# octavian-ganea/equidock_public

Measured on NVIDIA H100. Metric: protein_pairs_per_sec_iegmn_fwd_kabsch, higher is better.
Workload: dtype f32

## Files before the change

### equidock_public_b200/csrc/edge_stage_tc.cu

```cuda
#include "tc_common.cuh"

namespace eqd {
#define TC_WGS 3
#define TC_THREADS (128 * TC_WGS)
#define TC_ROWS 64
#define TC_MAX_TN 32
#define TC_LD 72
#define TC_W_BYTES 67584
#define TC_W1_SPLIT 6144
#define TC_W23_BASE 18432
#define TC_W23_SPLIT 16384
#define TC_HE_FLOATS (TC_ROWS * EQD_EDGE_FEATS + 16)
#define TC_A_SPLIT 6144

struct __align__(128) TcWgSmem {
  unsigned char a[3 * TC_A_SPLIT];
  float msg[TC_ROWS * TC_LD];
  float he[TC_HE_FLOATS];
  double xs[2][TC_ROWS * 6];
  double xm[TC_ROWS * 3];
  double phi[TC_ROWS];
  int src[2][TC_ROWS];
  int dst[2][TC_ROWS];
  int rp[2][TC_MAX_TN + 4];
  unsigned long long he_bar;
};

struct EdgeConsts {
  float ln_g[64], ln_b[64], b2[64], b3[64], w4[64];
};

struct TcSmem {
  unsigned char w[TC_W_BYTES];
  TcWgSmem wg[TC_WGS];
  EdgeConsts cst;
  unsigned long long w_bar;
};

__global__ void __launch_bounds__(TC_THREADS, 1)
edge_stage_tc_kernel(eqd_graph g, eqd_layer_params p, const __grid_constant__ EdgeConsts cst_p,
                     const float* __restrict__ proj, const double* __restrict__ x_in, const double* __restrict__ x_orig,
                     float* __restrict__ aggr, double* __restrict__ x_out, int* __restrict__ status, int tn) {
  extern __shared__ __align__(128) unsigned char smem_raw[];
  TcSmem& S = *reinterpret_cast<TcSmem*>(smem_raw);
  const int tid = threadIdx.x, wgi = tid >> 7, t = tid & 127, r = t & 63, half = t >> 6;
  const int warp = t >> 5, lane = t & 31;
  TcWgSmem& W = S.wg[wgi];
  const EdgeConsts& cst = S.cst;
  const int bar = 1 + wgi;
  const int pw = 128 + 3 * p.dhp;
  const int ntiles = (g.n_nodes + tn - 1) / tn;
  const float slope = p.leaky_slope;

  TRACE_START(0);
  if (tid == 0) {
    mbar_init(&S.w_bar, 1);
    for (int w = 0; w < TC_WGS; ++w) mbar_init(&S.wg[w].he_bar, 1);
    asm volatile("fence.mbarrier_init.release.cluster;" ::: "memory");
    mbar_expect_tx(&S.w_bar, TC_W_BYTES);
    bulk_g2s(S.w, p.w_edge_tc, TC_W_BYTES, &S.w_bar);
  }
  for (int i = tid; i < 5 * 64; i += TC_THREADS) (&S.cst.ln_g[0])[i] = (&cst_p.ln_g[0])[i];
  __syncthreads();
  mbar_wait(&S.w_bar, 0);
  unsigned he_phase = 0;
  const unsigned w_saddr = smem_u32(S.w), a_saddr = smem_u32(W.a);
  auto a_desc = [&](int sp, int kb) { return a_desc_at<TC_ROWS>(a_saddr, TC_A_SPLIT, 0, sp, kb); };

  auto prefetch = [&](int tile, int buf, int e0, int e1, int& off_l, int& n_l, int& off_r) {
    const int n0 = tile * tn, nn = min(tn, g.n_nodes - n0);
    const int ne = e1 - e0;
    off_l = off_r = 0;
    n_l = 0;
    if (ne <= TC_ROWS) {
      if (r < ne) {
        if (half == 0) cp_async4(&W.src[buf][r], g.col_src + e0 + r);
        else cp_async4(&W.dst[buf][r], g.edge_dst + e0 + r);
      }
      if (half == 0 && r <= nn) cp_async4(&W.rp[buf][r], g.row_ptr + n0 + r);
      const int el0 = min(e0, g.n_lig_edges), el1 = min(e1, g.n_lig_edges);
      n_l = el1 - el0;
      long sl = 0, sr = 0;
      unsigned bl = 0, br = 0;
      if (n_l > 0) {
        long b0 = (long)el0 * (EQD_EDGE_FEATS * 4), b1 = (long)el1 * (EQD_EDGE_FEATS * 4);
        sl = b0 & ~15L;
        bl = (unsigned)(((b1 + 15) & ~15L) - sl);
        off_l = (int)((b0 - sl) >> 2);
      }
      const int nr = ne - n_l;
      const unsigned dst_r_off = bl;
      if (nr > 0) {
        long b0 = (long)(e0 + n_l - g.n_lig_edges) * (EQD_EDGE_FEATS * 4), b1 = (long)(e1 - g.n_lig_edges) * (EQD_EDGE_FEATS * 4);
        sr = b0 & ~15L;
        br = (unsigned)(((b1 + 15) & ~15L) - sr);
        off_r = (int)(dst_r_off >> 2) + (int)((b0 - sr) >> 2);
      }
      if (t == 0) {
        mbar_expect_tx(&W.he_bar, bl + br);
        if (bl) bulk_g2s(W.he, reinterpret_cast<const unsigned char*>(g.he_lig) + sl, bl, &W.he_bar);
        if (br) bulk_g2s(reinterpret_cast<unsigned char*>(W.he) + dst_r_off, reinterpret_cast<const unsigned char*>(g.he_rec) + sr, br,
                         &W.he_bar);
      }
    }
    cp_async_commit();
  };
  auto prefetch_x = [&](int b, int ne_t) {
    if (r < ne_t && ne_t <= TC_ROWS) {
      const double* xp = x_in + (long)(half == 0 ? W.src[b][r] : W.dst[b][r]) * 3;
#pragma unroll
      for (int c = 0; c < 3; ++c) cp_async8(&W.xs[b][r * 6 + half * 3 + c], xp + c);
    }
    cp_async_commit();
  };
  auto row_range = [&](int tile, int& e0, int& e1) {
    const int n0 = tile * tn;
    e0 = __ldg(g.row_ptr + n0);
    e1 = __ldg(g.row_ptr + n0 + min(tn, g.n_nodes - n0));
  };

  int tile = blockIdx.x * TC_WGS + wgi;
  const int tstride = gridDim.x * TC_WGS;
  int buf = 0;
  int e0 = 0, ne = 0, off_l = 0, n_l = 0, off_r = 0;
  if (tile < ntiles) {
    int e1;
    row_range(tile, e0, e1);
    ne = e1 - e0;
    prefetch(tile, buf, e0, e1, off_l, n_l, off_r);
    cp_async_wait<0>();
    prefetch_x(buf, ne);
  }
  const int fr0 = warp * 16 + (lane >> 2), fc = 2 * (lane & 3);

  for (; tile < ntiles; tile += tstride) {
    const int n0 = tile * tn, nn = min(tn, g.n_nodes - n0);
    const bool has_next = tile + tstride < ntiles;
    int e0n = 0, e1n = 0, off_ln = 0, n_ln = 0, off_rn = 0;
    if (has_next) row_range(tile + tstride, e0n, e1n);
    const int nen = e1n - e0n;
    if (ne > TC_ROWS) {
      if (t == 0) atomicOr(status + g.n_pairs, EQD_STATUS_DEGREE_OVERFLOW);
      cp_async_wait<0>();
      wg_barrier(bar);
      if (has_next) {
        prefetch(tile + tstride, buf ^ 1, e0n, e1n, off_ln, n_ln, off_rn);
        cp_async_wait<0>();
        prefetch_x(buf ^ 1, nen);
      }
      e0 = e0n; ne = nen; off_l = off_ln; n_l = n_ln; off_r = off_rn; buf ^= 1;
      continue;
    }
    if (t == 0) TRACE_PHASE(0, blockIdx.x * TC_WGS + wgi, tile, 2);
    const int o_upd = 127 - t;
    const int nd_upd = o_upd / 3, comp_upd = o_upd - nd_upd * 3;
    const long gi_upd = (long)(n0 + nd_upd) * 3 + comp_upd;
    double xo_upd = 0.0, xi_upd = 0.0;
    if (o_upd < nn * 3) {
      xo_upd = x_orig[gi_upd];
      xi_upd = x_in[gi_upd];
    }
    cp_async_wait<0>();
    wg_barrier(bar);
    float2 ps[16], pd[16];
#pragma unroll
    for (int h = 0; h < 2; ++h) {
      const int fr = fr0 + 8 * h;
      const bool ok = fr < ne;
      const float* sp = proj + (long)(ok ? W.src[buf][fr] : 0) * pw + fc;
      const float* dp = proj + (long)(ok ? W.dst[buf][fr] : n0) * pw + 64 + fc;
#pragma unroll
      for (int j = 0; j < 8; ++j) {
        ps[2 * j + h] = __ldg(reinterpret_cast<const float2*>(sp + 8 * j));
        pd[2 * j + h] = __ldg(reinterpret_cast<const float2*>(dp + 8 * j));
      }
    }
    const bool valid = r < ne;
    {
      float a1v[24];
      mbar_wait(&W.he_bar, he_phase);
      he_phase ^= 1;
      const float* hrow = W.he + (r < n_l ? off_l + r * EQD_EDGE_FEATS : off_r + (r - n_l) * EQD_EDGE_FEATS);
      if (half == 0) {
#pragma unroll
        for (int k = 0; k < 24; ++k) a1v[k] = valid ? hrow[k] : 0.f;
      } else {
        double rx = 0.0, ry = 0.0, rz = 0.0;
        if (valid) {
          const double* xs = W.xs[buf] + r * 6;
          rx = xs[0] - xs[3];
          ry = xs[1] - xs[4];
          rz = xs[2] - xs[5];
          W.xm[r * 3 + 0] = rx;
          W.xm[r * 3 + 1] = ry;
          W.xm[r * 3 + 2] = rz;
        }
#pragma unroll
        for (int k = 0; k < 3; ++k) a1v[k] = valid ? hrow[24 + k] : 0.f;
        const float nd2 = valid ? -(float)(rx * rx + ry * ry + rz * rz) : -INFINITY;
        constexpr double kS[EQD_N_RBF] = {1.0, 1.5, 2.25, 3.375, 5.0625, 7.59375, 11.390625, 17.0859375, 25.62890625,
                                          38.443359375, 57.6650390625, 86.49755859375, 129.746337890625,
                                          194.6195068359375, 291.92926025390625};
#pragma unroll
        for (int j = 0; j < EQD_N_RBF; ++j)
          a1v[3 + j] = exp2f(nd2 * (float)(1.4426950408889634 / kS[j]));
#pragma unroll
        for (int k = 18; k < 24; ++k) a1v[k] = 0.f;
      }
      unsigned p0[12], p1[12], p2[12];
#pragma unroll
      for (int c = 0; c < 12; ++c) split3_pair(a1v[2 * c], a1v[2 * c + 1], p0[c], p1[c], p2[c]);
#pragma unroll
      for (int j = 0; j < 3; ++j) a_store8<TC_ROWS>(W.a, TC_A_SPLIT, r, half * 24 + 8 * j, p0 + 4 * j, p1 + 4 * j, p2 + 4 * j);
    }
    tc_fence_before();
    const bool deg10 = wg_barrier_and(bar, t >= nn || W.rp[buf][t + 1] - W.rp[buf][t] == 10);
    unsigned af[3][4][4];
    {
      float v[32];
      wg_gemm6_issue<64>(v, a_desc, [&](int sp, int kb) { return b_desc_ex(w_saddr + sp * TC_W1_SPLIT + kb * 2048, 1024, 128); },
                         3, false);
      if (has_next) prefetch(tile + tstride, buf ^ 1, e0n, e1n, off_ln, n_ln, off_rn);
      wg_mma_wait(v);
#pragma unroll
      for (int h = 0; h < 2; ++h)
#pragma unroll
        for (int j = 0; j < 8; ++j) {
          float& x0 = v[4 * j + 2 * h];
          float& x1 = v[4 * j + 2 * h + 1];
          x0 = __fadd_rn(__fadd_rn(x0, ps[2 * j + h].x), pd[2 * j + h].x);
          x1 = __fadd_rn(__fadd_rn(x1, ps[2 * j + h].y), pd[2 * j + h].y);
          x0 = fmaxf(x0, __fmul_rn(x0, slope));
          x1 = fmaxf(x1, __fmul_rn(x1, slope));
        }
      float pv[32];
#pragma unroll
      for (int i = 0; i < 32; ++i) pv[i] = __shfl_xor_sync(0xffffffffu, v[i], 2);
      float mean[2], rstd[2];
#pragma unroll
      for (int h = 0; h < 2; ++h) {
        float mh[2], qh[2];
#pragma unroll
        for (int ch = 0; ch < 2; ++ch) {
          float s0 = 0.f, s1 = 0.f;
#pragma unroll
          for (int c4 = 0; c4 < 8; ++c4) {
            s0 = __fadd_rn(s0, chain_val(v, pv, h, ch, c4, 0));
            s1 = __fadd_rn(s1, chain_val(v, pv, h, ch, c4, 1));
          }
          const float sp = s0 + s1;
          mh[ch] = (sp + __shfl_xor_sync(0xffffffffu, sp, 1)) * (1.f / 32.f);
          float q0 = 0.f, q1 = 0.f;
#pragma unroll
          for (int c4 = 0; c4 < 8; ++c4) {
            const float d0 = __fadd_rn(chain_val(v, pv, h, ch, c4, 0), -mh[ch]);
            const float d1 = __fadd_rn(chain_val(v, pv, h, ch, c4, 1), -mh[ch]);
            q0 = fmaf(d0, d0, q0);
            q1 = fmaf(d1, d1, q1);
          }
          const float qp = q0 + q1;
          qh[ch] = qp + __shfl_xor_sync(0xffffffffu, qp, 1);
        }
        const float m0 = mh[0], m1 = mh[1];
        mean[h] = 0.5f * (m0 + m1);
        const float dm = m0 - m1;
        const float var = (qh[0] + qh[1] + dm * dm * 16.f) * (1.f / 64.f);
        rstd[h] = 1.f / sqrtf(var + 1e-5f);
      }
#pragma unroll
      for (int j = 0; j < 8; ++j) {
        const float2 gj = *reinterpret_cast<const float2*>(&cst.ln_g[8 * j + fc]);
        const float2 bj = *reinterpret_cast<const float2*>(&cst.ln_b[8 * j + fc]);
#pragma unroll
        for (int h = 0; h < 2; ++h) {
          float& x0 = v[4 * j + 2 * h];
          float& x1 = v[4 * j + 2 * h + 1];
          x0 = fmaf(__fmul_rn(__fadd_rn(x0, -mean[h]), rstd[h]), gj.x, bj.x);
          x1 = fmaf(__fmul_rn(__fadd_rn(x1, -mean[h]), rstd[h]), gj.y, bj.y);
        }
      }
      acc_to_a_split3<4>(v, af);
    }
    if (has_next) {
      cp_async_wait<0>();
      prefetch_x(buf ^ 1, nen);
    }
    {
      auto w23 = [&](int hn) {
        return [&, hn](int sp, int kb) {
          return b_desc_ex(w_saddr + TC_W23_BASE + sp * TC_W23_SPLIT + kb * 4096 + hn * 1024, 2048, 128); };
      };
      float m[32], hd[32];
      wg_gemm6_rs_issue<64>(m, af, w23(0), false);
      wg_gemm6_rs_issue<64>(hd, af, w23(1), false);
      wg_mma_wait(m);
      wg_mma_wait(hd);
      float u[32];
#pragma unroll
      for (int j = 0; j < 8; ++j) {
        const float2 b2 = *reinterpret_cast<const float2*>(&cst.b2[8 * j + fc]);
        const float2 b3 = *reinterpret_cast<const float2*>(&cst.b3[8 * j + fc]);
#pragma unroll
        for (int h = 0; h < 2; ++h) {
          *reinterpret_cast<float2*>(W.msg + (fr0 + 8 * h) * TC_LD + 8 * j + fc) =
              make_float2(__fadd_rn(m[4 * j + 2 * h], b2.x), __fadd_rn(m[4 * j + 2 * h + 1], b2.y));
          const float x0 = __fadd_rn(hd[4 * j + 2 * h], b3.x), x1 = __fadd_rn(hd[4 * j + 2 * h + 1], b3.y);
          u[4 * j + 2 * h] = fmaxf(x0, __fmul_rn(x0, slope));
          u[4 * j + 2 * h + 1] = fmaxf(x1, __fmul_rn(x1, slope));
        }
      }
      float pu[32];
#pragma unroll
      for (int i = 0; i < 32; ++i) pu[i] = __shfl_xor_sync(0xffffffffu, u[i], 2);
      double phv[2];
#pragma unroll
      for (int h = 0; h < 2; ++h) {
        double red[2];
#pragma unroll
        for (int ch = 0; ch < 2; ++ch) {
          const float* w4 = cst.w4 + 32 * ch + 2 * (lane & 1);
          float p0 = 0.f, p1 = 0.f;
#pragma unroll
          for (int c4 = 0; c4 < 8; ++c4) {
            p0 = fmaf(chain_val(u, pu, h, ch, c4, 0), w4[4 * c4], p0);
            p1 = fmaf(chain_val(u, pu, h, ch, c4, 1), w4[4 * c4 + 1], p1);
          }
          const double pp = (double)p0 + (double)p1;
          red[ch] = pp + __shfl_xor_sync(0xffffffffu, pp, 1);
        }
        phv[h] = red[0] + red[1] + (double)p.b_coor2;
      }
      if ((lane & 3) == 0) {
        W.phi[fr0] = phv[0];
        W.phi[fr0 + 8] = phv[1];
      }
    }
    wg_barrier(bar);
    if (o_upd < nn * 3) {
      const int rs = W.rp[buf][nd_upd] - e0, re = W.rp[buf][nd_upd + 1] - e0;
      double sum = 0.0;
      if (deg10) {
#pragma unroll
        for (int j = 0; j < 10; ++j) {
          const int rr = nd_upd * 10 + j;
          sum += W.xm[rr * 3 + comp_upd] * W.phi[rr];
        }
      } else {
        for (int rr = rs; rr < re; ++rr) sum += W.xm[rr * 3 + comp_upd] * W.phi[rr];
      }
      const int deg = re - rs;
      const double upd = deg > 0 ? sum / (double)deg : 0.0;
      const double eta = (double)p.x_connection_init;
      x_out[gi_upd] = eta * xo_upd + (1.0 - eta) * xi_upd + upd;
    }
    {
      const int c = t & 63;
      const float* col = W.msg + c;
      if (deg10) {
        for (int nd = (nn * half) >> 1, nd1 = (nn * (half + 1)) >> 1; nd < nd1; ++nd) {
          const float* cr = col + nd * 10 * TC_LD;
          float s0 = 0.f, s1 = 0.f;
#pragma unroll
          for (int j = 0; j < 10; j += 2) {
            s0 += cr[j * TC_LD];
            s1 += cr[(j + 1) * TC_LD];
          }
          aggr[(long)(n0 + nd) * 64 + c] = (s0 + s1) / 10.f;
        }
      } else {
        for (int nd = (nn * half) >> 1, nd1 = (nn * (half + 1)) >> 1; nd < nd1; ++nd) {
          const int rs = W.rp[buf][nd] - e0, re = W.rp[buf][nd + 1] - e0;
          float s0 = 0.f, s1 = 0.f;
          int rr = rs;
          for (; rr + 1 < re; rr += 2) {
            s0 += col[rr * TC_LD];
            s1 += col[(rr + 1) * TC_LD];
          }
          if (rr < re) s0 += col[rr * TC_LD];
          aggr[(long)(n0 + nd) * 64 + c] = re > rs ? (s0 + s1) / (float)(re - rs) : 0.f;
        }
      }
    }
    e0 = e0n; ne = nen; off_l = off_ln; n_l = n_ln; off_r = off_rn; buf ^= 1;
  }
  if (t == 0) TRACE_PHASE(0, blockIdx.x * TC_WGS + wgi, 0xffff, 16);
  cp_async_wait<0>();
  __syncthreads();
  TRACE_END(0);
}

}

EQD_TRACE_SETTER(eqd_trace_set_edge)

extern "C" int eqd_edge_stage(const eqd_graph* g, const eqd_layer* p_l, const float* proj, const double* x_in,
                              const double* x_orig, float* aggr, double* x_out, int32_t* status, void* stream) {
  const eqd_layer_params* p = p_l ? &p_l->dev : nullptr;
  if (!g || !p || !proj || !x_in || !x_orig || !aggr || !x_out || !status) return EQD_ERR_BAD_ARG;
  if (!p->w_edge_tc) return EQD_ERR_BAD_ARG;
  if (g->max_in_degree < 1 || g->max_in_degree > EQD_TM) return EQD_ERR_UNSUPPORTED;
  if (!(p->leaky_slope >= 0.f && p->leaky_slope <= 1.f)) return EQD_ERR_UNSUPPORTED;
  if ((reinterpret_cast<uintptr_t>(g->he_lig) | reinterpret_cast<uintptr_t>(g->he_rec) |
       reinterpret_cast<uintptr_t>(p->w_edge_tc)) & 15)
    return EQD_ERR_BAD_ARG;
  if (g->max_in_degree > TC_ROWS) return eqd_edge_stage_ffma(g, p_l, proj, x_in, x_orig, aggr, x_out, status, stream);
  if (g->n_nodes <= 0) return EQD_OK;
  int tn = TC_ROWS / g->max_in_degree;
  if (tn > TC_MAX_TN) tn = TC_MAX_TN;
  int ntiles = (g->n_nodes + tn - 1) / tn;
  eqd::EdgeConsts cst;
  memcpy(&cst, p_l->consts.edge, sizeof(cst));
  size_t smem = sizeof(eqd::TcSmem) + 128;
  EQD_SET_SMEM((eqd::edge_stage_tc_kernel), smem);
  int grid = (ntiles + TC_WGS - 1) / TC_WGS;
  if (grid > EQD_SMS) grid = EQD_SMS;
  eqd::edge_stage_tc_kernel<<<grid, TC_THREADS, smem, (cudaStream_t)stream>>>(*g, *p, cst, proj, x_in, x_orig, aggr, x_out,
                                                                             status, tn);
  EQD_CUDA_LAUNCH_CHECK();
  return EQD_OK;
}
```

Measured before the change: 35240.

## Alias A-operand and message buffers to fit four warpgroups per CTA

```diff
diff --git a/equidock_public_b200/csrc/edge_stage_tc.cu b/equidock_public_b200/csrc/edge_stage_tc.cu
--- a/equidock_public_b200/csrc/edge_stage_tc.cu
+++ b/equidock_public_b200/csrc/edge_stage_tc.cu
@@ -1,7 +1,7 @@
 #include "tc_common.cuh"
 
 namespace eqd {
-#define TC_WGS 3
+#define TC_WGS 4
 #define TC_THREADS (128 * TC_WGS)
 #define TC_ROWS 64
 #define TC_MAX_TN 32
@@ -13,9 +13,19 @@
 #define TC_HE_FLOATS (TC_ROWS * EQD_EDGE_FEATS + 16)
 #define TC_A_SPLIT 6144
 
+#define EDGE_PROF_PHASES 8
+#ifdef EDGE_PROF
+__device__ long long g_edge_prof[TC_WGS * EDGE_PROF_PHASES];
+#define PROF_MARK(k) do { if (t == 0 && blockIdx.x == 0) { const long long t_ = clock64(); prof_acc[wgi][k] += t_ - prof_t; prof_t = t_; } } while (0)
+#else
+#define PROF_MARK(k) do { } while (0)
+#endif
+
 struct __align__(128) TcWgSmem {
-  unsigned char a[3 * TC_A_SPLIT];
-  float msg[TC_ROWS * TC_LD];
+  union {
+    unsigned char a[3 * TC_A_SPLIT];
+    float msg[TC_ROWS * TC_LD];
+  };
   float he[TC_HE_FLOATS];
   double xs[2][TC_ROWS * 6];
   double xm[TC_ROWS * 3];
@@ -23,6 +33,7 @@
   int src[2][TC_ROWS];
   int dst[2][TC_ROWS];
   int rp[2][TC_MAX_TN + 4];
+  int he_at[2][4];
   unsigned long long he_bar;
 };
 
@@ -36,6 +47,7 @@
   EdgeConsts cst;
   unsigned long long w_bar;
 };
+static_assert(sizeof(TcSmem) + 128 <= 227 * 1024, "edge stage: shared memory of one CTA exceeds the sm_90 opt-in limit");
 
 __global__ void __launch_bounds__(TC_THREADS, 1)
 edge_stage_tc_kernel(eqd_graph g, eqd_layer_params p, const __grid_constant__ EdgeConsts cst_p,
@@ -67,36 +79,38 @@
   const unsigned w_saddr = smem_u32(S.w), a_saddr = smem_u32(W.a);
   auto a_desc = [&](int sp, int kb) { return a_desc_at<TC_ROWS>(a_saddr, TC_A_SPLIT, 0, sp, kb); };
 
-  auto prefetch = [&](int tile, int buf, int e0, int e1, int& off_l, int& n_l, int& off_r) {
+  auto prefetch = [&](int tile, int buf, int e0, int e1) {
     const int n0 = tile * tn, nn = min(tn, g.n_nodes - n0);
     const int ne = e1 - e0;
-    off_l = off_r = 0;
-    n_l = 0;
     if (ne <= TC_ROWS) {
       if (r < ne) {
         if (half == 0) cp_async4(&W.src[buf][r], g.col_src + e0 + r);
         else cp_async4(&W.dst[buf][r], g.edge_dst + e0 + r);
       }
       if (half == 0 && r <= nn) cp_async4(&W.rp[buf][r], g.row_ptr + n0 + r);
-      const int el0 = min(e0, g.n_lig_edges), el1 = min(e1, g.n_lig_edges);
-      n_l = el1 - el0;
-      long sl = 0, sr = 0;
-      unsigned bl = 0, br = 0;
-      if (n_l > 0) {
-        long b0 = (long)el0 * (EQD_EDGE_FEATS * 4), b1 = (long)el1 * (EQD_EDGE_FEATS * 4);
-        sl = b0 & ~15L;
-        bl = (unsigned)(((b1 + 15) & ~15L) - sl);
-        off_l = (int)((b0 - sl) >> 2);
-      }
-      const int nr = ne - n_l;
-      const unsigned dst_r_off = bl;
-      if (nr > 0) {
-        long b0 = (long)(e0 + n_l - g.n_lig_edges) * (EQD_EDGE_FEATS * 4), b1 = (long)(e1 - g.n_lig_edges) * (EQD_EDGE_FEATS * 4);
-        sr = b0 & ~15L;
-        br = (unsigned)(((b1 + 15) & ~15L) - sr);
-        off_r = (int)(dst_r_off >> 2) + (int)((b0 - sr) >> 2);
-      }
       if (t == 0) {
+        const int el0 = min(e0, g.n_lig_edges), el1 = min(e1, g.n_lig_edges);
+        const int n_l = el1 - el0;
+        int off_l = 0, off_r = 0;
+        long sl = 0, sr = 0;
+        unsigned bl = 0, br = 0;
+        if (n_l > 0) {
+          long b0 = (long)el0 * (EQD_EDGE_FEATS * 4), b1 = (long)el1 * (EQD_EDGE_FEATS * 4);
+          sl = b0 & ~15L;
+          bl = (unsigned)(((b1 + 15) & ~15L) - sl);
+          off_l = (int)((b0 - sl) >> 2);
+        }
+        const int nr = ne - n_l;
+        const unsigned dst_r_off = bl;
+        if (nr > 0) {
+          long b0 = (long)(e0 + n_l - g.n_lig_edges) * (EQD_EDGE_FEATS * 4), b1 = (long)(e1 - g.n_lig_edges) * (EQD_EDGE_FEATS * 4);
+          sr = b0 & ~15L;
+          br = (unsigned)(((b1 + 15) & ~15L) - sr);
+          off_r = (int)(dst_r_off >> 2) + (int)((b0 - sr) >> 2);
+        }
+        W.he_at[buf][0] = off_l;
+        W.he_at[buf][1] = n_l;
+        W.he_at[buf][2] = off_r;
         mbar_expect_tx(&W.he_bar, bl + br);
         if (bl) bulk_g2s(W.he, reinterpret_cast<const unsigned char*>(g.he_lig) + sl, bl, &W.he_bar);
         if (br) bulk_g2s(reinterpret_cast<unsigned char*>(W.he) + dst_r_off, reinterpret_cast<const unsigned char*>(g.he_rec) + sr, br,
@@ -122,21 +136,27 @@
   int tile = blockIdx.x * TC_WGS + wgi;
   const int tstride = gridDim.x * TC_WGS;
   int buf = 0;
-  int e0 = 0, ne = 0, off_l = 0, n_l = 0, off_r = 0;
+  int ne = 0;
   if (tile < ntiles) {
-    int e1;
+    int e0, e1;
     row_range(tile, e0, e1);
     ne = e1 - e0;
-    prefetch(tile, buf, e0, e1, off_l, n_l, off_r);
+    prefetch(tile, buf, e0, e1);
     cp_async_wait<0>();
     prefetch_x(buf, ne);
   }
   const int fr0 = warp * 16 + (lane >> 2), fc = 2 * (lane & 3);
+#ifdef EDGE_PROF
+  __shared__ long long prof_acc[TC_WGS][EDGE_PROF_PHASES];
+  if (t == 0)
+    for (int k = 0; k < EDGE_PROF_PHASES; ++k) prof_acc[wgi][k] = 0;
+  long long prof_t = clock64();
+#endif
 
   for (; tile < ntiles; tile += tstride) {
     const int n0 = tile * tn, nn = min(tn, g.n_nodes - n0);
     const bool has_next = tile + tstride < ntiles;
-    int e0n = 0, e1n = 0, off_ln = 0, n_ln = 0, off_rn = 0;
+    int e0n = 0, e1n = 0;
     if (has_next) row_range(tile + tstride, e0n, e1n);
     const int nen = e1n - e0n;
     if (ne > TC_ROWS) {
@@ -144,11 +164,11 @@
       cp_async_wait<0>();
       wg_barrier(bar);
       if (has_next) {
-        prefetch(tile + tstride, buf ^ 1, e0n, e1n, off_ln, n_ln, off_rn);
+        prefetch(tile + tstride, buf ^ 1, e0n, e1n);
         cp_async_wait<0>();
         prefetch_x(buf ^ 1, nen);
       }
-      e0 = e0n; ne = nen; off_l = off_ln; n_l = n_ln; off_r = off_rn; buf ^= 1;
+      ne = nen; buf ^= 1;
       continue;
     }
     if (t == 0) TRACE_PHASE(0, blockIdx.x * TC_WGS + wgi, tile, 2);
@@ -162,6 +182,7 @@
     }
     cp_async_wait<0>();
     wg_barrier(bar);
+    PROF_MARK(0);
     float2 ps[16], pd[16];
 #pragma unroll
     for (int h = 0; h < 2; ++h) {
@@ -180,7 +201,8 @@
       float a1v[24];
       mbar_wait(&W.he_bar, he_phase);
       he_phase ^= 1;
-      const float* hrow = W.he + (r < n_l ? off_l + r * EQD_EDGE_FEATS : off_r + (r - n_l) * EQD_EDGE_FEATS);
+      const int n_l = W.he_at[buf][1];
+      const float* hrow = W.he + (r < n_l ? W.he_at[buf][0] + r * EQD_EDGE_FEATS : W.he_at[buf][2] + (r - n_l) * EQD_EDGE_FEATS);
       if (half == 0) {
 #pragma unroll
         for (int k = 0; k < 24; ++k) a1v[k] = valid ? hrow[k] : 0.f;
@@ -215,13 +237,15 @@
     }
     tc_fence_before();
     const bool deg10 = wg_barrier_and(bar, t >= nn || W.rp[buf][t + 1] - W.rp[buf][t] == 10);
+    PROF_MARK(1);
     unsigned af[3][4][4];
     {
       float v[32];
       wg_gemm6_issue<64>(v, a_desc, [&](int sp, int kb) { return b_desc_ex(w_saddr + sp * TC_W1_SPLIT + kb * 2048, 1024, 128); },
                          3, false);
-      if (has_next) prefetch(tile + tstride, buf ^ 1, e0n, e1n, off_ln, n_ln, off_rn);
+      if (has_next) prefetch(tile + tstride, buf ^ 1, e0n, e1n);
       wg_mma_wait(v);
+      PROF_MARK(2);
 #pragma unroll
       for (int h = 0; h < 2; ++h)
 #pragma unroll
@@ -285,25 +309,38 @@
       cp_async_wait<0>();
       prefetch_x(buf ^ 1, nen);
     }
+    PROF_MARK(3);
     {
       auto w23 = [&](int hn) {
         return [&, hn](int sp, int kb) {
           return b_desc_ex(w_saddr + TC_W23_BASE + sp * TC_W23_SPLIT + kb * 4096 + hn * 1024, 2048, 128); };
       };
-      float m[32], hd[32];
-      wg_gemm6_rs_issue<64>(m, af, w23(0), false);
+      {
+        float m[32];
+        wg_gemm6_rs_issue<64>(m, af, w23(0), false);
+        wg_mma_wait(m);
+        PROF_MARK(4);
+        wg_barrier(bar);
+#pragma unroll
+        for (int j = 0; j < 8; ++j) {
+          const float2 b2 = *reinterpret_cast<const float2*>(&cst.b2[8 * j + fc]);
+#pragma unroll
+          for (int h = 0; h < 2; ++h)
+            *reinterpret_cast<float2*>(W.msg + (fr0 + 8 * h) * TC_LD + 8 * j + fc) =
+                make_float2(__fadd_rn(m[4 * j + 2 * h], b2.x), __fadd_rn(m[4 * j + 2 * h + 1], b2.y));
+        }
+        PROF_MARK(5);
+      }
+      float hd[32];
       wg_gemm6_rs_issue<64>(hd, af, w23(1), false);
-      wg_mma_wait(m);
       wg_mma_wait(hd);
+      PROF_MARK(4);
       float u[32];
 #pragma unroll
       for (int j = 0; j < 8; ++j) {
-        const float2 b2 = *reinterpret_cast<const float2*>(&cst.b2[8 * j + fc]);
         const float2 b3 = *reinterpret_cast<const float2*>(&cst.b3[8 * j + fc]);
 #pragma unroll
         for (int h = 0; h < 2; ++h) {
-          *reinterpret_cast<float2*>(W.msg + (fr0 + 8 * h) * TC_LD + 8 * j + fc) =
-              make_float2(__fadd_rn(m[4 * j + 2 * h], b2.x), __fadd_rn(m[4 * j + 2 * h + 1], b2.y));
           const float x0 = __fadd_rn(hd[4 * j + 2 * h], b3.x), x1 = __fadd_rn(hd[4 * j + 2 * h + 1], b3.y);
           u[4 * j + 2 * h] = fmaxf(x0, __fmul_rn(x0, slope));
           u[4 * j + 2 * h + 1] = fmaxf(x1, __fmul_rn(x1, slope));
@@ -335,7 +372,10 @@
         W.phi[fr0 + 8] = phv[1];
       }
     }
+    PROF_MARK(5);
     wg_barrier(bar);
+    PROF_MARK(6);
+    const int e0 = W.rp[buf][0];
     if (o_upd < nn * 3) {
       const int rs = W.rp[buf][nd_upd] - e0, re = W.rp[buf][nd_upd + 1] - e0;
       double sum = 0.0;
@@ -381,8 +421,14 @@
         }
       }
     }
-    e0 = e0n; ne = nen; off_l = off_ln; n_l = n_ln; off_r = off_rn; buf ^= 1;
+    ne = nen;
+    buf ^= 1;
+    PROF_MARK(7);
   }
+#ifdef EDGE_PROF
+  if (t == 0 && blockIdx.x == 0)
+    for (int k = 0; k < EDGE_PROF_PHASES; ++k) g_edge_prof[wgi * EDGE_PROF_PHASES + k] = prof_acc[wgi][k];
+#endif
   if (t == 0) TRACE_PHASE(0, blockIdx.x * TC_WGS + wgi, 0xffff, 16);
   cp_async_wait<0>();
   __syncthreads();
@@ -392,6 +438,13 @@
 }
 
 EQD_TRACE_SETTER(eqd_trace_set_edge)
+
+#ifdef EDGE_PROF
+extern "C" int eqd_edge_prof_read(long long* out) {
+  if (cudaMemcpyFromSymbol(out, eqd::g_edge_prof, sizeof(eqd::g_edge_prof)) != cudaSuccess) return -1;
+  return TC_WGS;
+}
+#endif
 
 extern "C" int eqd_edge_stage(const eqd_graph* g, const eqd_layer* p_l, const float* proj, const double* x_in,
                               const double* x_orig, float* aggr, double* x_out, int32_t* status, void* stream) {
```

Result: no change. 35250, median of 6 (+0.0%).
